# pacellie/raytracer_challenge

Hardware: AMD Instinct MI355X
Metric: Mrays/s (unique rays: primary+shadow+reflection+refraction) at 1920x1080 depth-5 (higher is better)
Workload: dtype f64

## Files before the change

### raytracer_challenge_amd/csrc/device_scene.h

```cpp
#pragma once
#include <stddef.h>
#include <stdint.h>

enum { OP_PRIM = 0, OP_GROUP = 1, OP_MESH = 2, OP_BVH = 3, OP_QUIRK = 4, OP_QGRID = 5, OP_CSG = 6, OP_CSG_END = 7 };

struct DOp {
  int32_t op, a, b, c;
  int32_t g;
  int32_t pad[3];
};

#define RTC_KOPS 12
#define RTC_KPLANES 6
struct DPlaneK {
  double row[4];
  int32_t prim;
  int32_t gcond;
  int32_t pad[2];
  double n[3];
};

struct DBvhNode {
  float lo0[3], hi0[3];
  float lo1[3], hi1[3];
// ... 146 lines not shown
  unsigned long long accel_nodes, group_tests, tri_tests, analytic_tests;
  unsigned long long knodes;
  unsigned long long kplanes;
  unsigned long long light_cells;
  unsigned long long kgroups;
  unsigned long long diag[64];
  unsigned long long nan_ts;
  unsigned long long guard;
  unsigned long long guard_claim;
  long long guard_info[8];
  unsigned long long wf_overflow;
};
#define RTC_STATS_LAUNCH_BYTES offsetof(DStats, nan_ts)

#define RTC_MAX_FUEL 16

#if defined(__HIPCC__) || defined(RTC_EMU)
#define RTC_HD __host__ __device__
#else
#define RTC_HD
#endif
static inline RTC_HD unsigned long long rtc_mix64(unsigned long long x) {
  x ^= x >> 33; x *= 0xff51afd7ed558ccdull; x ^= x >> 33; x *= 0xc4ceb9fe1a85ec53ull; x ^= x >> 33;
  return x;
}
static inline RTC_HD unsigned long long rtc_hit_hash_base(unsigned long long t_bits, int32_t prim, int32_t push) {
  return rtc_mix64(t_bits) ^ ((((unsigned long long)(uint32_t)prim << 32) | (unsigned long long)(uint32_t)push) * 0x9E3779B97F4A7C15ull);
}
static inline RTC_HD unsigned long long rtc_hit_hash(unsigned long long base, int depth, int kind) {
  return rtc_mix64(base ^ ((unsigned long long)(((unsigned)depth << 8) | (unsigned)kind) + 1ull) * 0xD6E8FEB86659FD93ull);
}

static inline RTC_HD unsigned long long rtc_splitmix64(unsigned long long z) {
  z = (z ^ (z >> 30)) * 0xbf58476d1ce4e5b9ull; z = (z ^ (z >> 27)) * 0x94d049bb133111ebull;
  return z ^ (z >> 31);
}
static inline RTC_HD unsigned long long rtc_area_hash(int light, double x, double y, double z) {
  unsigned long long bx, by, bz;
  __builtin_memcpy(&bx, &x, 8); __builtin_memcpy(&by, &y, 8); __builtin_memcpy(&bz, &z, 8);
  return rtc_splitmix64(rtc_splitmix64(rtc_splitmix64(rtc_splitmix64((unsigned long long)(uint32_t)light) ^ bx) ^ by) ^ bz);
}
static inline RTC_HD double rtc_area_jitter(unsigned long long h, unsigned j) {
  return (double)(rtc_splitmix64(h ^ (unsigned long long)j) >> 11) * 0x1.0p-53;
}
#define RTC_ALIGHT 16

#define RTC_WF_SHADE_COUNT 32
#define RTC_WF_OVERFLOW 63
#define RTC_WF_CHUNK_NEXT 64
#define RTC_WF_COUNTS (64 + 32 * 8 * (RTC_MAX_FUEL + 2))
#ifndef RTC_WF_CHUNK
#define RTC_WF_CHUNK 64u
#endif
#define RTC_WF_MISS (-2)
struct DWave {
  double* rq[2];
  double* h_t;
  int32_t* h_prim;
  double* h_n12;
  double* sr;
  int32_t* sr_mat;
  int32_t* sr_node;
  double* contrib;
  int32_t* child;
  uint32_t* counts;
  uint32_t cap;
  uint32_t pad;
  unsigned long long* dig;
};
static inline uint64_t dwave_bytes(uint64_t cap, int levels) {
  return cap * (uint64_t)(7 + 7 + 1 + 2 + 9 + 3 * levels) * sizeof(double) + (cap * (uint64_t)(1 + 1 + 1 + 2 * levels) + RTC_WF_COUNTS) * sizeof(int32_t);
}
static inline void dwave_carve(DWave* W, void* mem, uint64_t cap, int levels) {
  double* d = (double*)mem;
  W->rq[0] = d; d += 7 * cap;
  W->rq[1] = d; d += 7 * cap;
  W->h_t = d; d += cap;
  W->h_n12 = d; d += 2 * cap;
  W->sr = d; d += 9 * cap;
  W->contrib = d; d += 3 * (uint64_t)levels * cap;
  int32_t* q = (int32_t*)d;
  W->h_prim = q; q += cap;
  W->sr_mat = q; q += cap;
  W->sr_node = q; q += cap;
  W->child = q; q += 2 * (uint64_t)levels * cap;
  W->counts = (uint32_t*)q;
  W->cap = (uint32_t)cap;
  W->pad = 0;
  W->dig = nullptr;
}
#ifndef RTC_BVH_STACK
#define RTC_BVH_STACK 64
#endif
```

### raytracer_challenge_amd/csrc/rtc_device.hpp

```cpp
#pragma once

#include <hip/hip_runtime.h>
#include <stdint.h>

#include <algorithm>

#include "device_scene.h"

#define EPS 0.00001
#ifndef RTC_BLOCK
#define RTC_BLOCK 64
#endif
#ifndef RTC_WAVES_PER_SIMD
#define RTC_WAVES_PER_SIMD 1
#endif
#ifdef RTC_TRAVERSE_NOINLINE
#define TRAVERSE_INLINE __noinline__
#else
#define TRAVERSE_INLINE __forceinline__
#endif
#ifndef RTC_LANE_ID
#define RTC_LANE_ID ((int)(threadIdx.x & 63u))
#endif
#ifndef RTC_WF_SHADE_BLOCK
// ... 1595 lines not shown
    K.tlo = -DINF; K.thi = T.best_t;
    K.c1_prim = -1; K.c2_prim = -1; K.c1_t = 0.0; K.c2_t = 0.0;
    DIAG_LOOP(19);
    {
      DIAG_SPAN_BEGIN();
#pragma unroll 1
      for (int rep_ = 0; rep_ < ((RTC_PROBE & 32) ? 2 : 1); rep_++) {
        Ray r2 = ray;
        if (RTC_PROBE & 32) RTC_LAUNDER(r2.ox);
        traverse<FEAT, KOPS, MODE_CONTAINERS, LDSC>(S, r2, K, C, stack, stride, L);
      }
      DIAG_SPAN_END(1);
    }
    if (K.c1_prim >= 0) n1 = S.mat[8 * S.prims[K.c1_prim].mat + 6];
    if (K.c2_prim >= 0) n2 = S.mat[8 * S.prims[K.c2_prim].mat + 6];
    W.h_n12[i] = n1; W.h_n12[cap + i] = n2;
  }
}

template <int FEAT, bool KOPS, bool LDSC>
__device__ __forceinline__ void wf_shadow_rec(const DScene& S, const DCamera& cam, const DPixelMap& pm, const DWave& W, const WorkMap& wm, int level, unsigned s, int* stack,
                                              int stride, Counters& C, unsigned& n_shadow, const LdsScene& L) {
  const size_t cap = W.cap;
  double* cb = W.contrib + (size_t)level * 3 * cap;
  const double* r = W.sr;
  const double px = r[s], py = r[cap + s], pz = r[2 * cap + s];
  unsigned long long shadow_mask = 0ull;
  for (int l = 0; l < S.n_lights; l++) {
    const double* LG = S.lights + 6 * l;
    double vx = LG[3] - px, vy = LG[4] - py, vz = LG[5] - pz;
    double distance = sqrt(vx * vx + vy * vy + vz * vz);
    Ray sray;
    sray.ox = px; sray.oy = py; sray.oz = pz;
    sray.dx = vx / distance; sray.dy = vy / distance; sray.dz = vz / distance;
    n_shadow++;
    Trav Sh;
    reset_closest(Sh, S.all_cast_shadow ? MODE_SHADOW_ANY : MODE_SHADOW_CLOSEST);
    if (S.all_cast_shadow) { Sh.thi = distance; Sh.unordered = 1; }
    Sh.light = l; Sh.c1_t = distance;
    DIAG_LOOP(18);
    DIAG_SPAN_BEGIN();
    if (S.all_cast_shadow) traverse<FEAT, KOPS, MODE_SHADOW_ANY, LDSC>(S, sray, Sh, C, stack, stride, L);
    else traverse<FEAT, KOPS, MODE_SHADOW_CLOSEST, LDSC>(S, sray, Sh, C, stack, stride, L);
    nan_commit(Sh, C);
    DIAG_SPAN_END(3);
    bool shadowed;
    if (S.all_cast_shadow) shadowed = Sh.shadowed != 0;
    else shadowed = (Sh.best_prim != 0x7fffffff) && (S.prims[Sh.best_prim].flags & 1u) && (Sh.best_t < distance);
    if (shadowed) shadow_mask |= 1ull << l;
  }
  DIAG_LOOP(20);
  DIAG_SPAN_BEGIN();
  const double nx = r[3 * cap + s], ny = r[4 * cap + s], nz = r[5 * cap + s];
  const double cr = r[6 * cap + s], cg = r[7 * cap + s], cbl = r[8 * cap + s];
  const int node = W.sr_node[s];
  double ex, ey, ez, weight;
  if (level == 0) {
    uint64_t q = 0;
    (void)work_to_slot(wm, (unsigned)node, q);
    const Ray pr = slot_ray(pm, cam, q);
    ex = -pr.dx; ey = -pr.dy; ez = -pr.dz; weight = 1.0;
  } else {
    const double* rq = W.rq[level & 1];
    ex = -rq[3 * cap + node]; ey = -rq[4 * cap + node]; ez = -rq[5 * cap + node]; weight = rq[6 * cap + node];
  }
  const double* M = S.mat + 8 * W.sr_mat[s];
  const double ambient = M[0], diffuse = M[1], specular = M[2], shininess = M[3];
  double sr = 0.0, sg = 0.0, sb = 0.0;
  for (int l = 0; l < S.n_lights * ((RTC_PROBE & 8) ? 2 : 1); l++) {
    if ((RTC_PROBE & 8) && l == S.n_lights) { sr = sg = sb = 0.0; }
    const int li = (RTC_PROBE & 8) ? l % S.n_lights : l;
    const double* LG = S.lights + 6 * li;
    double vx = LG[3] - px, vy = LG[4] - py, vz = LG[5] - pz;
    if (RTC_PROBE & 8) RTC_LAUNDER(vx);
    double distance = sqrt(vx * vx + vy * vy + vz * vz);
    const double ldx = vx / distance, ldy = vy / distance, ldz = vz / distance;
    const bool shadowed = (shadow_mask >> li) & 1ull;
    double er = cr * LG[0], eg = cg * LG[1], eb = cbl * LG[2];
    double lr = er * ambient, lg = eg * ambient, lb = eb * ambient;
    double ldn = ldx * nx + ldy * ny + ldz * nz;
    double dr = 0.0, dg = 0.0, db = 0.0, pr = 0.0, pg = 0.0, pb = 0.0;
    if (!shadowed && ldn >= 0.0) {
      dr = er * diffuse * ldn; dg = eg * diffuse * ldn; db = eb * diffuse * ldn;
      double mlx = -ldx, mly = -ldy, mlz = -ldz;
      double d2 = 2.0 * (mlx * nx + mly * ny + mlz * nz);
      double rfx = mlx - nx * d2, rfy = mly - ny * d2, rfz = mlz - nz * d2;
      double rde = rfx * ex + rfy * ey + rfz * ez;
      if (rde > 0.0) {
        double f = specular_factor(rde, shininess, specular);
        pr = LG[0] * specular * f; pg = LG[1] * specular * f; pb = LG[2] * specular * f;
      }
    }
    sr += (lr + dr) + pr; sg += (lg + dg) + pg; sb += (lb + db) + pb;
  }
  cb[node] = weight * sr; cb[cap + node] = weight * sg; cb[2 * cap + node] = weight * sb;
  DIAG_SPAN_END(5);
}

template <int FEAT, bool KOPS, bool LDSC>
__device__ __forceinline__ void wf_shadow_rec_area(const DScene& S, const DCamera& cam, const DPixelMap& pm, const DWave& W, const WorkMap& wm, int level, unsigned s,
                                                   int* stack, int stride, Counters& C, unsigned& n_shadow, const LdsScene& L) {
  const size_t cap = W.cap;
  double* cb = W.contrib + (size_t)level * 3 * cap;
  const double* r = W.sr;
  const int node = W.sr_node[s];
  double ex, ey, ez, weight;
  if (level == 0) {
    uint64_t q = 0;
    (void)work_to_slot(wm, (unsigned)node, q);
    const Ray pr = slot_ray(pm, cam, q);
    ex = -pr.dx; ey = -pr.dy; ez = -pr.dz; weight = 1.0;
  } else {
    const double* rq = W.rq[level & 1];
    ex = -rq[3 * cap + node]; ey = -rq[4 * cap + node]; ez = -rq[5 * cap + node]; weight = rq[6 * cap + node];
  }
  const double* M = S.mat + 8 * W.sr_mat[s];
  double sr = 0.0, sg = 0.0, sb = 0.0;
  shade_lights_area<FEAT, KOPS, LDSC, false>(S, r[s], r[cap + s], r[2 * cap + s], r[3 * cap + s], r[4 * cap + s], r[5 * cap + s], ex, ey, ez, r[6 * cap + s],
                                             r[7 * cap + s], r[8 * cap + s], M[0], M[1], M[2], M[3], C, stack, stride, n_shadow, L, sr, sg, sb);
  cb[node] = weight * sr; cb[cap + node] = weight * sg; cb[2 * cap + node] = weight * sb;
}

#ifndef RTC_WF_TS_WAVES
#define RTC_WF_TS_WAVES 3
#endif
#ifndef RTC_WF_TS_WAVES_MAXFEAT
#define RTC_WF_TS_WAVES_MAXFEAT 1
#endif
#ifndef RTC_LDS_BLOCK
#define RTC_LDS_BLOCK (256 * RTC_WF_TS_WAVES)
#endif
template <bool COUNT, int FEAT, bool KOPS, bool LDSC = false, bool AREA = false>
__global__ void __launch_bounds__(LDSC ? RTC_LDS_BLOCK : RTC_BLOCK, (KOPS || FEAT <= RTC_WF_TS_WAVES_MAXFEAT) ? RTC_WF_TS_WAVES : 2) wf_ts(DScene S, DCamera cam, DPixelMap pm, DWave W, int tl, int sl, unsigned n0, int slot, int fuel_left,
                                                                     double* __restrict__ hit_t, int* __restrict__ hit_prim, int* __restrict__ hit_k, DStats* __restrict__ stats) {
  RTC_LDS_STACK(lds_stack);
  LdsScene L = {nullptr, nullptr, nullptr, nullptr, 0, 0, 0};
  int* stack = lds_stack + threadIdx.x;
  int stride = RTC_BLOCK;
#ifndef RTC_EMU
  if (LDSC) {
    stack = (int*)lds_fill(S, (char*)lds_stack, L) + threadIdx.x;
    stride = (int)blockDim.x;
  }
#endif
  Counters C = {0, 0, 0, 0, 0, 0, 0, 0, 0};
  unsigned n_rays = 0, n_container = 0, n_shadow = 0;
#ifdef RTC_DIAG
  if (threadIdx.x < 64) s_diag[threadIdx.x] = 0ull;
  __syncthreads();
#endif
  const WorkMap wm = make_workmap(pm, cam);
  const unsigned nt = tl >= 0 ? wf_count(W, tl, n0) : 0u;
  unsigned ns = sl >= 0 ? W.counts[RTC_WF_SHADE_COUNT + sl] : 0u;
  if (ns > W.cap) ns = W.cap;
  const unsigned ct = (nt + RTC_WF_CHUNK - 1) / RTC_WF_CHUNK, cs = (ns + RTC_WF_CHUNK - 1) / RTC_WF_CHUNK;
  const unsigned nx = gridDim.x < 8u ? gridDim.x : 8u;
  const unsigned x = blockIdx.x % nx;
  unsigned* next = &W.counts[RTC_WF_CHUNK_NEXT + 32 * (8 * slot + (int)x)];
  const int lane = RTC_LANE_ID;
  for (;;) {
    unsigned kx = 0;
    if (lane == 0) kx = atomicAdd(next, 1u);
    kx = __shfl(kx, 0);
    const unsigned long long chunk = (unsigned long long)kx * nx + x;
    if (chunk >= (unsigned long long)ct + cs) break;
    if (chunk < ct) {
      const unsigned base = (unsigned)chunk * RTC_WF_CHUNK;
      for (unsigned o = 0; o < RTC_WF_CHUNK; o += RTC_WF_LANES) {
        const unsigned i = base + o + (unsigned)lane;
        if (i < nt) {
          DIAG_SPAN_BEGIN();
          wf_trace_ray<FEAT, KOPS, LDSC>(S, cam, pm, W, wm, tl, i, hit_t, hit_prim, hit_k, stack, stride, C, n_rays, n_container, fuel_left, L, COUNT && W.dig != nullptr);
// ... 95 lines not shown
```

### raytracer_challenge_amd/csrc/rtc_kernels.hip

```cpp
#include <cstdio>
#include <cstdlib>
#include <utility>

#include "rtc_device.hpp"

#ifdef RTC_EMU
#include "rtc_feat.hip"
constexpr int RTC_VARIANTS_BUILT = 6;
#else
constexpr int RTC_VARIANTS_BUILT = RTC_N_VARIANTS;
#endif
template <int... V>
static const RtcVariantOps& rtc_ops(int v, std::integer_sequence<int, V...>) {
  static const RtcVariantOps ops[RTC_N_VARIANTS] = {rtc_variant_ops<V>()...};
  return ops[v];
}
static const RtcVariantOps& rtc_ops(int v) { return rtc_ops(v, std::make_integer_sequence<int, RTC_VARIANTS_BUILT>{}); }
static int rtc_variant(const DScene& S, bool wavefront) {
  const int feat = S.has_csg ? 3 : (S.has_groups == 2 ? 2 : (S.has_groups ? 1 : 0));
  return rtc_pick_variant(feat, S.n_kops > 0, S.has_area != 0, S.has_uv != 0, wavefront);
}

#ifndef RTC_WF_SHADE_WAVES
#define RTC_WF_SHADE_WAVES 4
#endif
template <bool COUNT, bool PAT = true, bool UV = false>
__global__ void __launch_bounds__(RTC_WF_SHADE_BLOCK, RTC_WF_SHADE_WAVES) wf_shade(DScene S, DCamera cam, DPixelMap pm, DWave W, int level, unsigned n0, int fuel0, DStats* __restrict__ stats) {
  __shared__ unsigned s_rec2[2][2][16], s_child2[2][3][16];
  unsigned parity = 0;
  const WorkMap wm = make_workmap(pm, cam);
  const unsigned count = wf_count(W, level, n0);
  const size_t cap = W.cap;
  const double L = (double)S.n_lights;
  const int fuel = fuel0 - level;
  unsigned n_reflect = 0, n_refract = 0;
  int32_t* ch = W.child + (size_t)level * 2 * cap;
  double* nq = W.rq[(level + 1) & 1];
  const int lane = RTC_LANE_ID;
  const int wave = (int)(threadIdx.x / (RTC_WF_SHADE_BLOCK >= 64 ? 64 : 1));
  const int n_waves = RTC_WF_SHADE_BLOCK >= 64 ? RTC_WF_SHADE_BLOCK / 64 : 1;
  for (unsigned base = blockIdx.x * RTC_WF_SHADE_BLOCK; base < count; base += gridDim.x * RTC_WF_SHADE_BLOCK) {
    const unsigned i = base + threadIdx.x;
    int prim = -1;
    if (i < count) prim = W.h_prim[i];
    const bool hit = prim >= 0;
    State st;
    double cr = 0.0, cg = 0.0, cbl = 0.0, weight = 1.0, n1 = 1.0, n2 = 1.0;
    int mat = 0, geom = 0;
    double reflective = 0.0, transparency = 0.0;
    if (hit) {
      Ray ray;
      if (level == 0) {
        uint64_t q = 0;
        (void)work_to_slot(wm, i, q);
        ray = slot_ray(pm, cam, q);
      } else {
        ray = wf_load_ray(W, level, i, weight);
      }
      const DPrim P = S.prims[prim];
      mat = P.mat;
      geom = P.geom;
      const double* M = S.mat + 8 * P.mat;
      reflective = M[4]; transparency = M[5];
      double hu, hv;
      hit_uv(S, P, ray, hu, hv);
      prepare_state(S, P, ray, W.h_t[i], hu, hv, st);
      if (transparency != 0.0 && fuel > 0) { n1 = W.h_n12[i]; n2 = W.h_n12[cap + i]; }
      const double* mi = S.xf_matinv + 16 * P.xform;
      double x = mi[0] * st.px + mi[1] * st.py + mi[2] * st.pz + mi[3] * 1.0;
      double y = mi[4] * st.px + mi[5] * st.py + mi[6] * st.pz + mi[7] * 1.0;
      double z = mi[8] * st.px + mi[9] * st.py + mi[10] * st.pz + mi[11] * 1.0;
      double w = mi[12] * st.px + mi[13] * st.py + mi[14] * st.pz + mi[15] * 1.0;
      const DPat& root = S.pats[S.mat_pattern[P.mat]];
      if (!PAT || root.tag == 1) { cr = root.color[0]; cg = root.color[1]; cbl = root.color[2]; }
      else if constexpr (UV) pattern_color_uv(S, S.mat_pattern[P.mat], x, y, z, w, cr, cg, cbl);
      else pattern_color(S, S.mat_pattern[P.mat], x, y, z, w, cr, cg, cbl);
    }
    const bool blend = hit && reflective > 0.0 && transparency > 0.0;
    double R = 0.0;
    if (blend) R = blend_reflectance(st, n1, n2, fuel, cr, cg, cbl);
    bool do_refl = false, do_refr = false;
    double wr = 0.0, wt = 0.0, tdx = 0.0, tdy = 0.0, tdz = 0.0;
    if (hit && fuel > 0) {
      do_refl = reflective != 0.0;
      do_refr = transparency != 0.0;
      wr = weight * L * reflective; wt = weight * L * transparency;
      if (blend) {
        wr *= R;
        wt *= (1.0 - R);
      }
      if (do_refr) {
        double n_ratio = n1 / n2;
        double cos_i = st.ex * st.nx + st.ey * st.ny + st.ez * st.nz;
        double sin2_t = (n_ratio * n_ratio) * (1.0 - cos_i * cos_i);
        if (sin2_t > 1.0) do_refr = false;
        else {
          double cos_t = sqrt(1.0 - sin2_t);
          double kk = n_ratio * cos_i - cos_t;
          tdx = st.nx * kk - st.ex * n_ratio; tdy = st.ny * kk - st.ey * n_ratio; tdz = st.nz * kk - st.ez * n_ratio;
        }
      }
    }
    const unsigned long long lt = (1ull << lane) - 1ull;
    const bool on_plane = hit && geom == 1;
    const unsigned long long m_rec0 = __ballot(hit && on_plane ? 1 : 0), m_rec1 = __ballot(hit && !on_plane ? 1 : 0);
    const unsigned long long m_c0 = __ballot(do_refl && on_plane ? 1 : 0), m_c1 = __ballot(do_refl && !on_plane ? 1 : 0), m_c2 = __ballot(do_refr ? 1 : 0);
    unsigned (*s_rec)[16] = s_rec2[parity];
    unsigned (*s_child)[16] = s_child2[parity];
    parity ^= 1u;
    if (lane == 0) {
      s_rec[0][wave] = (unsigned)__popcll(m_rec0); s_rec[1][wave] = (unsigned)__popcll(m_rec1);
      s_child[0][wave] = (unsigned)__popcll(m_c0); s_child[1][wave] = (unsigned)__popcll(m_c1); s_child[2][wave] = (unsigned)__popcll(m_c2);
    }
    __syncthreads();
    if (threadIdx.x == 0) {
      unsigned tr = 0, tc = 0;
      for (int w = 0; w < n_waves; w++) { tr += s_rec[0][w] + s_rec[1][w]; tc += s_child[0][w] + s_child[1][w] + s_child[2][w]; }
      unsigned br = tr ? atomicAdd(&W.counts[RTC_WF_SHADE_COUNT + level], tr) : 0u;
      unsigned bc = tc ? atomicAdd(&W.counts[level + 1], tc) : 0u;
      if ((unsigned long long)br + tr > W.cap || (unsigned long long)bc + tc > W.cap) { W.counts[RTC_WF_OVERFLOW] = 1u; stats->wf_overflow = 1ull; }
      for (int k = 0; k < 2; k++)
        for (int w = 0; w < n_waves; w++) { unsigned r = s_rec[k][w]; s_rec[k][w] = br; br += r; }
      for (int k = 0; k < 3; k++)
        for (int w = 0; w < n_waves; w++) { unsigned c = s_child[k][w]; s_child[k][w] = bc; bc += c; }
    }
    __syncthreads();
    const unsigned s = on_plane ? s_rec[0][wave] + (unsigned)__popcll(m_rec0 & lt) : s_rec[1][wave] + (unsigned)__popcll(m_rec1 & lt);
    const unsigned jr = on_plane ? s_child[0][wave] + (unsigned)__popcll(m_c0 & lt) : s_child[1][wave] + (unsigned)__popcll(m_c1 & lt);
    const unsigned jt = s_child[2][wave] + (unsigned)__popcll(m_c2 & lt);
    if (hit && s < W.cap) {
      double* r = W.sr;
      r[s] = st.px; r[cap + s] = st.py; r[2 * cap + s] = st.pz;
      r[3 * cap + s] = st.nx; r[4 * cap + s] = st.ny; r[5 * cap + s] = st.nz;
      r[6 * cap + s] = cr; r[7 * cap + s] = cg; r[8 * cap + s] = cbl;
      W.sr_mat[s] = mat;
      W.sr_node[s] = (int32_t)i;
    }
    if (do_refl && jr < W.cap) {
      nq[jr] = st.px; nq[cap + jr] = st.py; nq[2 * cap + jr] = st.pz; nq[3 * cap + jr] = st.rx; nq[4 * cap + jr] = st.ry; nq[5 * cap + jr] = st.rz;
      nq[6 * cap + jr] = wr;
      ch[i] = (int32_t)jr;
      n_reflect++;
    }
    if (do_refr && jt < W.cap) {
      nq[jt] = st.ux; nq[cap + jt] = st.uy; nq[2 * cap + jt] = st.uz; nq[3 * cap + jt] = tdx; nq[4 * cap + jt] = tdy; nq[5 * cap + jt] = tdz;
      nq[6 * cap + jt] = wt;
      ch[cap + i] = (int32_t)jt;
      n_refract++;
    }
  }
  if (COUNT) {
    atomicAdd(&stats->rays_reflect, (unsigned long long)n_reflect);
    atomicAdd(&stats->rays_refract, (unsigned long long)n_refract);
  }
}

__global__ void __launch_bounds__(256) wf_gather(DCamera cam, DPixelMap pm, DWave W, unsigned n0, double* __restrict__ rgb) {
  const WorkMap wm = make_workmap(pm, cam);
  const size_t cap = W.cap;
  for (unsigned i = blockIdx.x * blockDim.x + threadIdx.x; i < n0; i += gridDim.x * blockDim.x) {
    uint64_t q;
    if (!work_to_slot(wm, i, q)) continue;
    double r = 0.0, g = 0.0, b = 0.0;
    int wait_idx[RTC_MAX_FUEL + 1];
    int wait_lvl[RTC_MAX_FUEL + 1];
    int sp = 0, lvl = 0, idx = (int)i;
    const bool digest = W.dig != nullptr && pm.digest != nullptr;
    unsigned long long dg = 0ull;
    int kind = 0;
    for (;;) {
      const double* cb = W.contrib + (size_t)lvl * 3 * cap;
      const int32_t* ch = W.child + (size_t)lvl * 2 * cap;
      const int a = ch[idx], c = ch[cap + idx];
      if (a != RTC_WF_MISS) { r += cb[idx]; g += cb[cap + idx]; b += cb[2 * cap + idx]; }
      if (digest) dg += rtc_hit_hash(W.dig[(size_t)lvl * cap + idx], lvl, kind);
      if (c >= 0) { wait_idx[sp] = c; wait_lvl[sp] = lvl + 1; sp++; }
      if (a >= 0) { idx = a; lvl++; kind = 1; continue; }
      if (sp == 0) break;
      sp--;
      idx = wait_idx[sp]; lvl = wait_lvl[sp]; kind = 2;
    }
    rgb[3 * q + 0] = r; rgb[3 * q + 1] = g; rgb[3 * q + 2] = b;
    if (digest) pm.digest[q] = dg;
  }
}


#ifndef RTC_EMU
unsigned rtc_wavefront_lds_bytes(const DScene& S) {
  static const bool off = [] { const char* e = std::getenv("RTC_WF_LDS"); return e && e[0] == '0'; }();
  if (off || !rtc_v_lds(RTC_VARIANTS[rtc_variant(S, true)])) return 0;
  const unsigned long long need = rtc_lds_table_bytes(S) + (unsigned long long)RTC_LDS_BLOCK * (unsigned)S.bvh_stack * sizeof(int);
  return need <= 158ull * 1024 ? (unsigned)need : 0u;
}

unsigned rtc_wavefront_grid(const DScene& S, int n_cu) {
  return (unsigned)std::max(1, n_cu * rtc_ops(rtc_variant(S, true)).wf_ts_blocks_per_cu(rtc_stack_bytes(S)));
}
#endif

uint64_t rtc_wavefront_work(const DCamera& cam, const DPixelMap& pm) {
  if (pm.mode == 2 && cam.hsize >= 8 && pm.n % cam.hsize == 0) return (uint64_t)((cam.hsize + 7) / 8) * ((pm.n / cam.hsize + 7) / 8) * 64;
  return pm.n;
}

void rtc_launch_wavefront(const DScene& S, const DCamera& cam, const DPixelMap& pm, int fuel, const DWave& W, double* rgb, double* hit_t, int* hit_prim, int* hit_k,
                          DStats* stats, bool count, hipStream_t stream, unsigned blocks, unsigned shade_blocks) {
  if (pm.n == 0) return;
  const RtcVariantOps& ops = rtc_ops(rtc_variant(S, true));
  const RtcFrame F = {S, cam, pm, hit_t, hit_prim, hit_k, stats, stream, count};
  const unsigned n0 = (unsigned)rtc_wavefront_work(cam, pm);
#ifndef RTC_EMU
  const unsigned lds = rtc_wavefront_lds_bytes(S);
  const unsigned lds_blocks = std::max(1u, shade_blocks / 2u);
#endif
  const dim3 sgrid(std::max(1u, shade_blocks)), sblock(RTC_WF_SHADE_BLOCK);
  for (int level = 0; level <= fuel + 1; level++) {
    const int tl = level <= fuel ? level : -1, sl = level - 1;
#ifndef RTC_EMU
    if (!lds || !ops.launch_wf_ts_lds(F, RtcLevel{W, tl, sl, n0, level, fuel - level, lds_blocks, lds}))
#endif
    ops.launch_wf_ts(F, RtcLevel{W, tl, sl, n0, level, fuel - level, blocks, 0u});
    if (level <= fuel) {
#ifndef RTC_EMU
      if (S.has_uv) {
        if (count) hipLaunchKernelGGL((wf_shade<true, true, true>), sgrid, sblock, 0, stream, S, cam, pm, W, level, n0, fuel, stats);
        else hipLaunchKernelGGL((wf_shade<false, true, true>), sgrid, sblock, 0, stream, S, cam, pm, W, level, n0, fuel, stats);
        continue;
      }
#endif
      if (count) hipLaunchKernelGGL((wf_shade<true>), sgrid, sblock, 0, stream, S, cam, pm, W, level, n0, fuel, stats);
      else if (S.all_plain) hipLaunchKernelGGL((wf_shade<false, false>), sgrid, sblock, 0, stream, S, cam, pm, W, level, n0, fuel, stats);
      else hipLaunchKernelGGL((wf_shade<false>), sgrid, sblock, 0, stream, S, cam, pm, W, level, n0, fuel, stats);
    }
  }
  hipLaunchKernelGGL(wf_gather, dim3(std::max(1u, std::min(blocks, (n0 + 255u) / 256u))), dim3(256), 0, stream, cam, pm, W, n0, rgb);
}

static dim3 rtc_elementwise_grid(unsigned long long n) { return dim3((unsigned)std::min<unsigned long long>((n + 255) / 256, 8192)); }
__global__ void __launch_bounds__(256) rtc_quantize_kernel(const double* __restrict__ rgb, unsigned char* __restrict__ out, unsigned long long n) {
  unsigned long long i = (unsigned long long)blockIdx.x * blockDim.x + threadIdx.x;
  const unsigned long long stride = (unsigned long long)gridDim.x * blockDim.x;
  for (; i < n; i += stride) {
    double x = rgb[i];
    double c = (x != x) ? 1.0 : (x < 1.0 ? x : 1.0);
    c = c > 0.0 ? c : 0.0;
    double r = round(c * 255.0);
    out[i] = (unsigned char)(r <= 0.0 ? 0.0 : (r >= 255.0 ? 255.0 : r));
  }
}
__global__ void __launch_bounds__(256) rtc_pack_hits_kernel(const double* __restrict__ t, const int* __restrict__ prim, const int* __restrict__ k, DHit* __restrict__ out, unsigned long long n) {
  for (unsigned long long i = (unsigned long long)blockIdx.x * blockDim.x + threadIdx.x; i < n; i += (unsigned long long)gridDim.x * blockDim.x) {
    DHit h;
    h.t = t[i]; h.prim = prim[i]; h.k = k[i];
    out[i] = h;
  }
}
void rtc_launch_pack_hits(const double* t, const int* prim, const int* k, DHit* out, unsigned long long n, hipStream_t stream) {
  if (n == 0) return;
  hipLaunchKernelGGL(rtc_pack_hits_kernel, rtc_elementwise_grid(n), dim3(256), 0, stream, t, prim, k, out, n);
}
void rtc_launch_quantize(const double* rgb, unsigned char* out, unsigned long long n, hipStream_t stream) {
  if (n == 0) return;
  hipLaunchKernelGGL(rtc_quantize_kernel, rtc_elementwise_grid(n), dim3(256), 0, stream, rgb, out, n);
}


template <typename T>
__global__ void __launch_bounds__(256) rtc_deinterleave_kernel(const T* __restrict__ slab, T* __restrict__ image, unsigned rowlen, unsigned vsize, unsigned n, unsigned max_rows,
                                                               unsigned band) {
  const unsigned long long total = (unsigned long long)vsize * rowlen;
  for (unsigned long long i = (unsigned long long)blockIdx.x * blockDim.x + threadIdx.x; i < total; i += (unsigned long long)gridDim.x * blockDim.x) {
    const unsigned y = (unsigned)(i / rowlen), x = (unsigned)(i % rowlen);
    const unsigned b = y / band;
    image[i] = slab[((unsigned long long)(b % n) * max_rows + (b / n) * band + y % band) * rowlen + x];
  }
}
template <typename T>
static void launch_deinterleave(const T* slab, T* image, unsigned rowlen, unsigned vsize, unsigned n, unsigned max_rows, unsigned band, hipStream_t stream) {
  const unsigned long long total = (unsigned long long)vsize * rowlen;
  if (total == 0) return;
  hipLaunchKernelGGL(rtc_deinterleave_kernel<T>, rtc_elementwise_grid(total), dim3(256), 0, stream, slab, image, rowlen, vsize, n, max_rows, band ? band : 1u);
}
void rtc_launch_deinterleave8(const unsigned char* slab, unsigned char* image, unsigned rowlen, unsigned vsize, unsigned n, unsigned max_rows, unsigned band, hipStream_t stream) {
  launch_deinterleave(slab, image, rowlen, vsize, n, max_rows, band, stream);
// ... 13 lines not shown
```

### raytracer_challenge_amd/csrc/scene_build.hpp

```cpp
#pragma once
#include <chrono>
#include <cstdio>
#include <algorithm>
#include <atomic>
#include <cmath>
#include <cstdlib>
#include <cstring>
#include <map>
#include <string>
#include <thread>
#include <vector>

#include "../../include/rtc.h"
#include "bvh_build.hpp"
#include "device_scene.h"
#include "host_scene.hpp"

namespace rtb {

template <class F>
inline void parallel_for(size_t n, size_t grain, F fn) {
  unsigned t = std::thread::hardware_concurrency();
  if (const char* e = std::getenv("RTC_BUILD_THREADS")) t = (unsigned)std::max(1, std::atoi(e));
  t = std::min<unsigned>(std::max(1u, t), 8u);
// ... 629 lines not shown
      o.pad[0] = -1;
      if ((o.op == OP_BVH || o.op == OP_MESH) && n_aux < RTC_KAUX && o.a >= 0) {
        DKAux& A = d.kaux[n_aux];
        std::memcpy(A.frame, &bvh_frame[(size_t)o.c * 4], 4 * sizeof(double));
        if (o.op == OP_MESH) std::memcpy(A.xf, &xf_inv[(size_t)o.b * 12], 12 * sizeof(double));
        else std::memset(A.xf, 0, sizeof(A.xf));
        A.root = bvh[(size_t)o.a];
        o.pad[0] = n_aux++;
      }
      if (o.op == OP_QGRID && !have_qgrid) { d.kqgrid = qgrids[(size_t)o.a]; have_qgrid = true; o.pad[0] = 0; }
      if (o.op == OP_PRIM && prims[(size_t)o.a].geom == RTC_PLANE && d.n_kplanes < RTC_KPLANES) {
        DPlaneK& k = d.kplanes[d.n_kplanes];
        std::memcpy(k.row, &xf_inv[(size_t)prims[(size_t)o.a].xform * 12 + 4], 4 * sizeof(double));
        k.prim = o.a;
        k.gcond = prims[(size_t)o.a].gcond;
        plane_world_normal(&xf_inv[(size_t)prims[(size_t)o.a].xform * 12], k.n);
        o.c = d.n_kplanes++;
      }
      d.kops[i] = o;
    }
    d.n_kops = (int32_t)ops.size();
  }

  DScene view() const {
    DScene d{};
    d.ops = ops.data(); d.group_box = group_box.data(); d.group_parent = group_parent.data(); d.bvh = bvh.data(); d.mtri = mtri.data(); d.mtri_prim = mtri_prim.data();
    d.item_prim = items.data(); d.quirk_prim = items.data(); d.qgrids = qgrids.data(); d.qcell = qcell.data(); d.bvh_frame = bvh_frame.data(); d.csg = csg.data(); d.qitem = items.data(); d.prims = prims.data(); d.pisect = pisect.data(); d.xf_inv = xf_inv.data(); d.xf_matinv = xf_matinv.data(); d.limits = limits.data();
    d.tri_geo = tri_geo.data(); d.tri_nrm = tri_nrm.data(); d.mat = mat.data(); d.mat_pattern = mat_pattern.data(); d.pats = pats.data();
    d.lights = lights.data();
    d.n_ops = (int32_t)ops.size(); d.n_prims = (int32_t)prims.size(); d.n_recs = (int32_t)pisect.size(); d.n_lights = n_lights; d.all_cast_shadow = all_cast_shadow;
    d.n_bvh = (int32_t)bvh.size(); d.n_items = (int32_t)items.size(); d.n_mtri = (int32_t)mtri_prim.size(); d.n_quirk = (int32_t)items.size();
    d.n_qitem = (int32_t)items.size(); d.n_qcell = (int32_t)qcell.size(); d.n_groups = (int32_t)(group_box.size() / 6); d.n_qgrids = (int32_t)qgrids.size();
    d.bvh_stack = bvh_stack;
    d.csg_max_hits = csg_max_hits;
    d.csg_slab = nullptr;
    d.has_mesh = 0;
    d.has_csg = 0;
    d.has_groups = 0;
    for (const DOp& o : ops) if (o.g >= 0) d.has_groups = 1;
    for (const DOp& o : ops) if ((o.op == OP_PRIM) && prims[o.a].gcond >= 0) d.has_groups = 2;
    for (size_t i = 0; i < std::min(items.size(), n_plain_items); i++) if (prims[items[i]].gcond >= 0) d.has_groups = 2;
    for (int32_t pi : bvh_prims) if (prims[pi].gcond >= 0) d.has_groups = 2;
    for (const DOp& o : ops) { if (o.op == OP_MESH) d.has_mesh = 1; if (o.op == OP_CSG) d.has_csg = 1; }
    fill_kernarg_program(d);
    d.quirk_reach2 = quirk_reach2;
    std::memcpy(d.abvh_frame, abvh_frame, sizeof(d.abvh_frame));
    d.light_grid_first = 0;
    for (const DOp& o : ops) if (o.op == OP_BVH && o.b > 0) d.light_grid_first = o.b;
    d.light_grid_n = 0; d.light_grid_cell_off = 0;
    if (d.light_grid_first > 0) { d.light_grid_n = qgrids[(size_t)d.light_grid_first - 1].n; d.light_grid_cell_off = qgrids[(size_t)d.light_grid_first - 1].cell_off; }
    d.all_plain = 1;
    for (int32_t root : mat_pattern) if (root < 0 || (size_t)root >= pats.size() || pats[(size_t)root].tag != 1) d.all_plain = 0;
    d.no_glass_mirror = 1;
    for (size_t m = 0; m + 7 < mat.size(); m += 8) if (mat[m + 4] != 0.0 && mat[m + 5] != 0.0) d.no_glass_mirror = 0;
    {
      const char* env = std::getenv("RTC_BACKFACE_SKIP");
      const bool on = !(env && env[0] == '0');
      auto bounded = [](const std::vector<double>& v) {
        std::atomic<bool> ok{true};
        parallel_for(v.size(), 1u << 20, [&](size_t b, size_t e) {
          for (size_t i = b; i < e; i++) if (!(std::fabs(v[i]) < 1e30)) { ok = false; return; }
        });
        return ok.load();
      };
      auto not_flat = [](const std::vector<double>& m) {
        for (size_t i = 0; i + 11 < m.size(); i += 12) {
          const double* r = &m[i];
          const double det = r[0] * (r[5] * r[10] - r[6] * r[9]) - r[1] * (r[4] * r[10] - r[6] * r[8]) + r[2] * (r[4] * r[9] - r[5] * r[8]);
          if (!(std::fabs(det) >= 1e-30)) return false;
        }
        return true;
      };
      if (backface_cached < 0) backface_cached = (bounded(xf_inv) && not_flat(xf_inv) && bounded(tri_geo) && bounded(lights) && area_bounded) ? 1 : 0;
      d.backface_skip = on ? backface_cached : 0;
    }
    d.has_area = has_area;
    d.has_uv = has_uv;
    d.has_recs = 0;
    for (size_t i = 0; i < ops.size(); i++) {
      const DOp& o = ops[i];
      if (o.op == OP_BVH || o.op == OP_QUIRK || o.op == OP_QGRID || o.op == OP_CSG) d.has_recs = 1;
      if (o.op == OP_PRIM && (d.n_kops == 0 || d.kops[i].c < 0)) d.has_recs = 1;
    }
    return d;
  }
};

inline int build_arrays(const rtc_scene_desc& D, HostArrays* H, std::string* err, bvh::DeviceBuildFn device_build = nullptr, size_t device_build_min = 4096,
                        const UvInput& uv = UvInput{}) {
  int rc = validate(D, err, uv);
  if (rc != RTC_OK) return rc;
  if (D.n_lights > 64) { *err = "more than 64 lights (the wavefront path keeps one shadow bit per light)"; return RTC_ERR_UNSUPPORTED; }
  const bool timing = std::getenv("RTC_TIMING") != nullptr;
  auto t_start = std::chrono::steady_clock::now();
  auto lap = [&](const char* what) {
    if (!timing) return;
    auto now = std::chrono::steady_clock::now();
    std::fprintf(stderr, "[rtc-timing] %-28s %.3f s\n", what, std::chrono::duration<double>(now - t_start).count());
    t_start = now;
  };
  lap("validate");
  ProgramBuilder pb{D};
  pb.device_build = device_build;
  pb.device_build_min = device_build_min;
  if (const char* e = std::getenv("RTC_CUBE_PAD")) pb.cube_pad = std::max(0.0, std::atof(e));
  for (uint32_t i = 0; i < D.n_prims && pb.cube_pad > 0.0; i++) {
    if (D.prims[i].geometry != RTC_CUBE) continue;
    rth::M4 inv = rth::M4::from(D.xforms[D.prims[i].xform].transform_inv), fwd;
    if (!inv.invert(&fwd)) { pb.cube_pad = 0.0; break; }
    for (int c = 0; c < 3; c++) {
      const double nrm = std::sqrt(fwd.a[0][c] * fwd.a[0][c] + fwd.a[1][c] * fwd.a[1][c] + fwd.a[2][c] * fwd.a[2][c]);
      if (!(nrm < 1e3)) pb.cube_pad = 0.0;
    }
  }
  if (const char* e = std::getenv("RTC_DEVICE_BVH_MIN")) pb.device_build_min = (size_t)std::strtoull(e, nullptr, 10);
  if (!pb.emit(0, D.n_nodes) || pb.status != RTC_OK) { *err = pb.error; return pb.status != RTC_OK ? pb.status : RTC_ERR_INVALID; }
  lap("program + BVH build");
  H->prims.resize(D.n_prims);
  std::atomic<int> all_cast{1};
  parallel_for(D.n_prims, 65536, [&](size_t b, size_t e) {
    int cast = 1;
    for (size_t i = b; i < e; i++) {
      H->prims[i] = {D.prims[i].geometry, D.prims[i].flags, D.prims[i].material, D.prims[i].xform, D.prims[i].data, pb.prim_gcond.empty() ? -1 : pb.prim_gcond[i], {0, 0}};
      if (!(D.prims[i].flags & RTC_FLAG_CASTS_SHADOW)) cast = 0;
    }
    if (!cast) all_cast.store(0);
  });
  H->all_cast_shadow = all_cast.load();
  H->xf_inv.resize((size_t)D.n_xforms * 12);
  H->xf_matinv.resize((size_t)D.n_xforms * 16);
  for (uint32_t i = 0; i < D.n_xforms; i++) {
    std::memcpy(&H->xf_inv[(size_t)i * 12], D.xforms[i].transform_inv, 12 * sizeof(double));
    std::memcpy(&H->xf_matinv[(size_t)i * 16], D.xforms[i].material_inv, 16 * sizeof(double));
  }
  H->limits.assign(D.limits, D.limits + (size_t)D.n_limits * 2);
  H->tri_geo.assign(D.tri_p1e1e2, D.tri_p1e1e2 + (size_t)D.n_tris * 9);
  H->tri_nrm.assign(D.tri_normals, D.tri_normals + (size_t)D.n_tris * 9);
  H->mat.assign((size_t)D.n_materials * 8, 0.0);
  H->mat_pattern.resize(D.n_materials);
  for (uint32_t i = 0; i < D.n_materials; i++) {
    const rtc_material& m = D.materials[i];
    double* q = &H->mat[(size_t)i * 8];
    q[0] = m.ambient; q[1] = m.diffuse; q[2] = m.specular; q[3] = m.shininess; q[4] = m.reflective; q[5] = m.transparency; q[6] = m.refractive_index;
    H->mat_pattern[i] = m.pattern;
  }
  H->pats.resize(D.n_pattern_nodes);
  for (uint32_t i = 0; i < D.n_pattern_nodes; i++) {
    const rtc_pattern_node& p = D.pattern_nodes[i];
    DPat& q = H->pats[i];
    std::memset(&q, 0, sizeof(q));
    q.tag = p.tag; q.kind = p.kind; q.noise_kind = p.noise_kind; q.octaves = p.octaves; q.left = p.left; q.right = p.right; q.scale = p.scale;
    std::memcpy(q.color, p.color, sizeof(q.color));
    std::memcpy(q.m, p.transform_inv, sizeof(q.m));
  }
  H->lights.resize((size_t)D.n_lights * 6);
  for (uint32_t i = 0; i < D.n_lights; i++) {
    std::memcpy(&H->lights[(size_t)i * 6], D.lights[i].intensity, 3 * sizeof(double));
    std::memcpy(&H->lights[(size_t)i * 6 + 3], D.lights[i].origin, 3 * sizeof(double));
  }
  H->n_lights = (int32_t)D.n_lights;
  for (const DPat& p : H->pats) if (p.tag == RTC_PAT_UV) H->has_uv = 1;
  if (H->has_uv) {
    const size_t rec0 = H->pats.size() * sizeof(DPat), tex0 = rec0 + (size_t)uv.n_pats * sizeof(DUv);
    std::vector<size_t> toff(uv.n_tex);
    size_t end = tex0;
    for (uint32_t t = 0; t < uv.n_tex; t++) { toff[t] = end; end += (size_t)3 * uv.tex[t].width * uv.tex[t].height * sizeof(double); }
    for (DPat& p : H->pats) if (p.tag == RTC_PAT_UV) p.uv = (int64_t)(rec0 + (size_t)p.left * sizeof(DUv));
    H->pats.resize((end + sizeof(DPat) - 1) / sizeof(DPat));
    char* base = (char*)H->pats.data();
    for (uint32_t k = 0; k < uv.n_pats; k++) {
      const rtc_uv_pattern& q = uv.pats[k];
      DUv o;
      std::memset(&o, 0, sizeof(o));
      o.kind = q.kind;
      std::memcpy(o.child, q.child, sizeof(o.child));
      o.width = q.width; o.height = q.height;
      if (q.kind == RTC_UV_IMAGE) { o.tw = (int32_t)uv.tex[q.texture].width; o.th = (int32_t)uv.tex[q.texture].height; o.off = (int64_t)toff[(size_t)q.texture]; }
      std::memcpy(base + rec0 + (size_t)k * sizeof(DUv), &o, sizeof(o));
    }
    for (uint32_t t = 0; t < uv.n_tex; t++) std::memcpy(base + toff[t], uv.tex[t].rgb, (size_t)3 * uv.tex[t].width * uv.tex[t].height * sizeof(double));
  }
  if (pb.ops.empty()) {
    pb.ops.push_back({OP_GROUP, 0, 1, 0, -1, {0, 0, 0}});
    pb.group_box.insert(pb.group_box.end(), {1, 1, 1, 0, 0, 0});
    pb.group_parent.push_back(-1);
  }
  lap("array copies");
  H->ops = std::move(pb.ops);
  H->group_box = std::move(pb.group_box);
  H->group_parent = std::move(pb.group_parent);
  H->bvh = std::move(pb.bvh_nodes);
  H->mtri = std::move(pb.mtri);
  H->mtri_prim = std::move(pb.mtri_prim);
  H->items = std::move(pb.items);
  H->n_plain_items = pb.n_plain_items;
  if (pb.have_abvh && pb.cube_pad > 0.0) {
    const double reach = pb.cube_pad / 0.00001;
// ... 101 lines not shown
```

Before: 11150.

## Pipeline wavefront shade loads, shrink plain-material shade records, and DPP-scan slot counters

```diff
diff --git a/raytracer_challenge_amd/csrc/device_scene.h b/raytracer_challenge_amd/csrc/device_scene.h
--- a/raytracer_challenge_amd/csrc/device_scene.h
+++ b/raytracer_challenge_amd/csrc/device_scene.h
@@ -222,6 +222,7 @@
 #ifndef RTC_WF_CHUNK
 #define RTC_WF_CHUNK 64u
 #endif
+#define RTC_SR_PLAIN 0x40000000
 #define RTC_WF_MISS (-2)
 struct DWave {
   double* rq[2];
diff --git a/raytracer_challenge_amd/csrc/rtc_device.hpp b/raytracer_challenge_amd/csrc/rtc_device.hpp
--- a/raytracer_challenge_amd/csrc/rtc_device.hpp
+++ b/raytracer_challenge_amd/csrc/rtc_device.hpp
@@ -1671,7 +1671,11 @@
   DIAG_LOOP(20);
   DIAG_SPAN_BEGIN();
   const double nx = r[3 * cap + s], ny = r[4 * cap + s], nz = r[5 * cap + s];
-  const double cr = r[6 * cap + s], cg = r[7 * cap + s], cbl = r[8 * cap + s];
+  const int mrow = W.sr_mat[s];
+  const double* M = S.mat + 8 * (mrow & (RTC_SR_PLAIN - 1));
+  double cr, cg, cbl;
+  if (mrow & RTC_SR_PLAIN) { cr = M[4]; cg = M[5]; cbl = M[6]; }
+  else { cr = r[6 * cap + s]; cg = r[7 * cap + s]; cbl = r[8 * cap + s]; }
   const int node = W.sr_node[s];
   double ex, ey, ez, weight;
   if (level == 0) {
@@ -1683,7 +1687,6 @@
     const double* rq = W.rq[level & 1];
     ex = -rq[3 * cap + node]; ey = -rq[4 * cap + node]; ez = -rq[5 * cap + node]; weight = rq[6 * cap + node];
   }
-  const double* M = S.mat + 8 * W.sr_mat[s];
   const double ambient = M[0], diffuse = M[1], specular = M[2], shininess = M[3];
   double sr = 0.0, sg = 0.0, sb = 0.0;
   for (int l = 0; l < S.n_lights * ((RTC_PROBE & 8) ? 2 : 1); l++) {
@@ -1733,10 +1736,14 @@
     const double* rq = W.rq[level & 1];
     ex = -rq[3 * cap + node]; ey = -rq[4 * cap + node]; ez = -rq[5 * cap + node]; weight = rq[6 * cap + node];
   }
-  const double* M = S.mat + 8 * W.sr_mat[s];
+  const int mrow = W.sr_mat[s];
+  const double* M = S.mat + 8 * (mrow & (RTC_SR_PLAIN - 1));
+  double cr, cg, cbl;
+  if (mrow & RTC_SR_PLAIN) { cr = M[4]; cg = M[5]; cbl = M[6]; }
+  else { cr = r[6 * cap + s]; cg = r[7 * cap + s]; cbl = r[8 * cap + s]; }
   double sr = 0.0, sg = 0.0, sb = 0.0;
-  shade_lights_area<FEAT, KOPS, LDSC, false>(S, r[s], r[cap + s], r[2 * cap + s], r[3 * cap + s], r[4 * cap + s], r[5 * cap + s], ex, ey, ez, r[6 * cap + s],
-                                             r[7 * cap + s], r[8 * cap + s], M[0], M[1], M[2], M[3], C, stack, stride, n_shadow, L, sr, sg, sb);
+  shade_lights_area<FEAT, KOPS, LDSC, false>(S, r[s], r[cap + s], r[2 * cap + s], r[3 * cap + s], r[4 * cap + s], r[5 * cap + s], ex, ey, ez, cr, cg, cbl, M[0], M[1], M[2],
+                                             M[3], C, stack, stride, n_shadow, L, sr, sg, sb);
   cb[node] = weight * sr; cb[cap + node] = weight * sg; cb[2 * cap + node] = weight * sb;
 }
 
diff --git a/raytracer_challenge_amd/csrc/rtc_kernels.hip b/raytracer_challenge_amd/csrc/rtc_kernels.hip
--- a/raytracer_challenge_amd/csrc/rtc_kernels.hip
+++ b/raytracer_challenge_amd/csrc/rtc_kernels.hip
@@ -24,9 +24,37 @@
 #ifndef RTC_WF_SHADE_WAVES
 #define RTC_WF_SHADE_WAVES 4
 #endif
-template <bool COUNT, bool PAT = true, bool UV = false>
+namespace {
+struct WfShadeIn {
+  int prim;
+  Ray ray;
+  double weight, t;
+};
+__device__ __forceinline__ int wf_shade_fetch_prim(const DWave& W, unsigned long long i, unsigned count) { return i < count ? W.h_prim[i] : -1; }
+template <bool LV0>
+__device__ __forceinline__ WfShadeIn wf_shade_prefetch(const DWave& W, int level, unsigned long long i, int lane, unsigned count, int prim) {
+  const unsigned long long first = i - (unsigned)lane;
+  const unsigned j = prim >= 0 ? (unsigned)i : (first < count ? (unsigned)first : 0u);
+  WfShadeIn in = {prim, {0.0, 0.0, 0.0, 0.0, 0.0, 0.0}, 1.0, 0.0};
+  if (!LV0) in.ray = wf_load_ray(W, level, j, in.weight);
+  in.t = W.h_t[j];
+  return in;
+}
+#ifndef RTC_EMU
+__device__ __forceinline__ unsigned wf_row_scan16(unsigned v) {
+  v += (unsigned)__builtin_amdgcn_update_dpp(0, (int)v, 0x111, 0xf, 0xf, true);
+  v += (unsigned)__builtin_amdgcn_update_dpp(0, (int)v, 0x112, 0xf, 0xf, true);
+  v += (unsigned)__builtin_amdgcn_update_dpp(0, (int)v, 0x114, 0xf, 0xf, true);
+  v += (unsigned)__builtin_amdgcn_update_dpp(0, (int)v, 0x118, 0xf, 0xf, true);
+  return v;
+}
+#endif
+}
+template <bool COUNT, bool PAT = true, bool UV = false, bool PIPE = false, bool LV0 = false>
 __global__ void __launch_bounds__(RTC_WF_SHADE_BLOCK, RTC_WF_SHADE_WAVES) wf_shade(DScene S, DCamera cam, DPixelMap pm, DWave W, int level, unsigned n0, int fuel0, DStats* __restrict__ stats) {
-  __shared__ unsigned s_rec2[2][2][16], s_child2[2][3][16];
+  constexpr int n_waves = RTC_WF_SHADE_BLOCK >= 64 ? RTC_WF_SHADE_BLOCK / 64 : 1;
+  static_assert(n_waves <= 8, "wf_shade: eight counters per class");
+  __shared__ unsigned s_cnt2[2][40];
   unsigned parity = 0;
   const WorkMap wm = make_workmap(pm, cam);
   const unsigned count = wf_count(W, level, n0);
@@ -38,47 +66,65 @@
   double* nq = W.rq[(level + 1) & 1];
   const int lane = RTC_LANE_ID;
   const int wave = (int)(threadIdx.x / (RTC_WF_SHADE_BLOCK >= 64 ? 64 : 1));
-  const int n_waves = RTC_WF_SHADE_BLOCK >= 64 ? RTC_WF_SHADE_BLOCK / 64 : 1;
-  for (unsigned base = blockIdx.x * RTC_WF_SHADE_BLOCK; base < count; base += gridDim.x * RTC_WF_SHADE_BLOCK) {
-    const unsigned i = base + threadIdx.x;
-    int prim = -1;
-    if (i < count) prim = W.h_prim[i];
+  const unsigned long long step = (unsigned long long)gridDim.x * RTC_WF_SHADE_BLOCK;
+  WfShadeIn nx = {-1, {0.0, 0.0, 0.0, 0.0, 0.0, 0.0}, 1.0, 0.0};
+  int nx_prim = -1;
+  const bool level0 = PIPE ? LV0 : level == 0;
+  if (PIPE) {
+    const unsigned long long i0 = (unsigned long long)blockIdx.x * RTC_WF_SHADE_BLOCK + threadIdx.x;
+    nx = wf_shade_prefetch<LV0>(W, level, i0, lane, count, wf_shade_fetch_prim(W, i0, count));
+  }
+  for (unsigned long long base = (unsigned long long)blockIdx.x * RTC_WF_SHADE_BLOCK; base < count; base += step) {
+    const unsigned i = (unsigned)base + threadIdx.x;
+    const WfShadeIn in = nx;
+    const int prim = PIPE ? in.prim : wf_shade_fetch_prim(W, i, count);
+    if (PIPE) nx_prim = wf_shade_fetch_prim(W, base + step + threadIdx.x, count);
     const bool hit = prim >= 0;
     State st;
     double cr = 0.0, cg = 0.0, cbl = 0.0, weight = 1.0, n1 = 1.0, n2 = 1.0;
-    int mat = 0, geom = 0;
+    int mat = 0, shading_row = 0, geom = 0;
     double reflective = 0.0, transparency = 0.0;
     if (hit) {
       Ray ray;
-      if (level == 0) {
+      if (level0) {
         uint64_t q = 0;
         (void)work_to_slot(wm, i, q);
         ray = slot_ray(pm, cam, q);
+      } else if (PIPE) {
+        ray = in.ray;
+        weight = in.weight;
       } else {
         ray = wf_load_ray(W, level, i, weight);
       }
       const DPrim P = S.prims[prim];
-      mat = P.mat;
       geom = P.geom;
       const double* M = S.mat + 8 * P.mat;
       reflective = M[4]; transparency = M[5];
+      mat = ~P.mat;
+      if (PIPE) shading_row = (int)M[7];
       double hu, hv;
       hit_uv(S, P, ray, hu, hv);
-      prepare_state(S, P, ray, W.h_t[i], hu, hv, st);
+      prepare_state(S, P, ray, PIPE ? in.t : W.h_t[i], hu, hv, st);
       if (transparency != 0.0 && fuel > 0) { n1 = W.h_n12[i]; n2 = W.h_n12[cap + i]; }
-      const double* mi = S.xf_matinv + 16 * P.xform;
-      double x = mi[0] * st.px + mi[1] * st.py + mi[2] * st.pz + mi[3] * 1.0;
-      double y = mi[4] * st.px + mi[5] * st.py + mi[6] * st.pz + mi[7] * 1.0;
-      double z = mi[8] * st.px + mi[9] * st.py + mi[10] * st.pz + mi[11] * 1.0;
-      double w = mi[12] * st.px + mi[13] * st.py + mi[14] * st.pz + mi[15] * 1.0;
-      const DPat& root = S.pats[S.mat_pattern[P.mat]];
-      if (!PAT || root.tag == 1) { cr = root.color[0]; cg = root.color[1]; cbl = root.color[2]; }
-      else if constexpr (UV) pattern_color_uv(S, S.mat_pattern[P.mat], x, y, z, w, cr, cg, cbl);
-      else pattern_color(S, S.mat_pattern[P.mat], x, y, z, w, cr, cg, cbl);
+      if constexpr (PAT) {
+        const double* mi = S.xf_matinv + 16 * P.xform;
+        double x = mi[0] * st.px + mi[1] * st.py + mi[2] * st.pz + mi[3] * 1.0;
+        double y = mi[4] * st.px + mi[5] * st.py + mi[6] * st.pz + mi[7] * 1.0;
+        double z = mi[8] * st.px + mi[9] * st.py + mi[10] * st.pz + mi[11] * 1.0;
+        double w = mi[12] * st.px + mi[13] * st.py + mi[14] * st.pz + mi[15] * 1.0;
+        if (S.pats[S.mat_pattern[P.mat]].tag != 1) {
+          if constexpr (UV) pattern_color_uv(S, S.mat_pattern[P.mat], x, y, z, w, cr, cg, cbl);
+          else pattern_color(S, S.mat_pattern[P.mat], x, y, z, w, cr, cg, cbl);
+          mat = P.mat;
+        }
+      }
     }
     const bool blend = hit && reflective > 0.0 && transparency > 0.0;
     double R = 0.0;
-    if (blend) R = blend_reflectance(st, n1, n2, fuel, cr, cg, cbl);
+    if (blend) {
+      R = blend_reflectance(st, n1, n2, fuel, cr, cg, cbl);
+      if (R != R && mat < 0) mat = ~mat;
+    }
     bool do_refl = false, do_refr = false;
     double wr = 0.0, wt = 0.0, tdx = 0.0, tdy = 0.0, tdz = 0.0;
     if (hit && fuel > 0) {
@@ -105,35 +151,57 @@
     const bool on_plane = hit && geom == 1;
     const unsigned long long m_rec0 = __ballot(hit && on_plane ? 1 : 0), m_rec1 = __ballot(hit && !on_plane ? 1 : 0);
     const unsigned long long m_c0 = __ballot(do_refl && on_plane ? 1 : 0), m_c1 = __ballot(do_refl && !on_plane ? 1 : 0), m_c2 = __ballot(do_refr ? 1 : 0);
-    unsigned (*s_rec)[16] = s_rec2[parity];
-    unsigned (*s_child)[16] = s_child2[parity];
+    unsigned* s_cnt = s_cnt2[parity];
     parity ^= 1u;
     if (lane == 0) {
-      s_rec[0][wave] = (unsigned)__popcll(m_rec0); s_rec[1][wave] = (unsigned)__popcll(m_rec1);
-      s_child[0][wave] = (unsigned)__popcll(m_c0); s_child[1][wave] = (unsigned)__popcll(m_c1); s_child[2][wave] = (unsigned)__popcll(m_c2);
-    }
+      s_cnt[wave] = (unsigned)__popcll(m_rec0); s_cnt[8 + wave] = (unsigned)__popcll(m_rec1);
+      s_cnt[16 + wave] = (unsigned)__popcll(m_c0); s_cnt[24 + wave] = (unsigned)__popcll(m_c1); s_cnt[32 + wave] = (unsigned)__popcll(m_c2);
+    }
+    if (PIPE) nx = wf_shade_prefetch<LV0>(W, level, base + step + threadIdx.x, lane, count, nx_prim);
     __syncthreads();
+#ifndef RTC_EMU
+    if (PIPE && n_waves == 8 && wave == 0) {
+      const unsigned c = lane < 40 ? s_cnt[lane] : 0u;
+      const unsigned in_row = wf_row_scan16(c);
+      const unsigned tr = (unsigned)__builtin_amdgcn_readlane((int)in_row, 15), t1 = (unsigned)__builtin_amdgcn_readlane((int)in_row, 31);
+      const unsigned tc = t1 + (unsigned)__builtin_amdgcn_readlane((int)in_row, 39);
+      const unsigned total = lane == 0 ? tr : tc;
+      unsigned old = 0u;
+      if (lane < 2 && total) {
+        old = atomicAdd(&W.counts[lane == 0 ? RTC_WF_SHADE_COUNT + level : level + 1], total);
+        if ((unsigned long long)old + total > W.cap) { W.counts[RTC_WF_OVERFLOW] = 1u; stats->wf_overflow = 1ull; }
+      }
+      const unsigned br = (unsigned)__builtin_amdgcn_readlane((int)old, 0), bc = (unsigned)__builtin_amdgcn_readlane((int)old, 1);
+      if (lane < 40) s_cnt[lane] = (lane < 16 ? br : bc + (lane >= 32 ? t1 : 0u)) + in_row - c;
+    }
+    if (!PIPE || n_waves != 8)
+#endif
     if (threadIdx.x == 0) {
       unsigned tr = 0, tc = 0;
-      for (int w = 0; w < n_waves; w++) { tr += s_rec[0][w] + s_rec[1][w]; tc += s_child[0][w] + s_child[1][w] + s_child[2][w]; }
+      for (int w = 0; w < n_waves; w++) { tr += s_cnt[w] + s_cnt[8 + w]; tc += s_cnt[16 + w] + s_cnt[24 + w] + s_cnt[32 + w]; }
       unsigned br = tr ? atomicAdd(&W.counts[RTC_WF_SHADE_COUNT + level], tr) : 0u;
       unsigned bc = tc ? atomicAdd(&W.counts[level + 1], tc) : 0u;
       if ((unsigned long long)br + tr > W.cap || (unsigned long long)bc + tc > W.cap) { W.counts[RTC_WF_OVERFLOW] = 1u; stats->wf_overflow = 1ull; }
       for (int k = 0; k < 2; k++)
-        for (int w = 0; w < n_waves; w++) { unsigned r = s_rec[k][w]; s_rec[k][w] = br; br += r; }
-      for (int k = 0; k < 3; k++)
-        for (int w = 0; w < n_waves; w++) { unsigned c = s_child[k][w]; s_child[k][w] = bc; bc += c; }
+        for (int w = 0; w < n_waves; w++) { unsigned r = s_cnt[8 * k + w]; s_cnt[8 * k + w] = br; br += r; }
+      for (int k = 2; k < 5; k++)
+        for (int w = 0; w < n_waves; w++) { unsigned c = s_cnt[8 * k + w]; s_cnt[8 * k + w] = bc; bc += c; }
     }
     __syncthreads();
-    const unsigned s = on_plane ? s_rec[0][wave] + (unsigned)__popcll(m_rec0 & lt) : s_rec[1][wave] + (unsigned)__popcll(m_rec1 & lt);
-    const unsigned jr = on_plane ? s_child[0][wave] + (unsigned)__popcll(m_c0 & lt) : s_child[1][wave] + (unsigned)__popcll(m_c1 & lt);
-    const unsigned jt = s_child[2][wave] + (unsigned)__popcll(m_c2 & lt);
+    const unsigned s = on_plane ? s_cnt[wave] + (unsigned)__popcll(m_rec0 & lt) : s_cnt[8 + wave] + (unsigned)__popcll(m_rec1 & lt);
+    const unsigned jr = on_plane ? s_cnt[16 + wave] + (unsigned)__popcll(m_c0 & lt) : s_cnt[24 + wave] + (unsigned)__popcll(m_c1 & lt);
+    const unsigned jt = s_cnt[32 + wave] + (unsigned)__popcll(m_c2 & lt);
     if (hit && s < W.cap) {
       double* r = W.sr;
       r[s] = st.px; r[cap + s] = st.py; r[2 * cap + s] = st.pz;
       r[3 * cap + s] = st.nx; r[4 * cap + s] = st.ny; r[5 * cap + s] = st.nz;
-      r[6 * cap + s] = cr; r[7 * cap + s] = cg; r[8 * cap + s] = cbl;
-      W.sr_mat[s] = mat;
+      if (mat >= 0) {
+        r[6 * cap + s] = cr; r[7 * cap + s] = cg; r[8 * cap + s] = cbl;
+        W.sr_mat[s] = mat;
+      } else {
+        if (!PIPE) shading_row = (int)S.mat[8 * ~mat + 7];
+        W.sr_mat[s] = RTC_SR_PLAIN | shading_row;
+      }
       W.sr_node[s] = (int32_t)i;
     }
     if (do_refl && jr < W.cap) {
@@ -230,7 +298,8 @@
       }
 #endif
       if (count) hipLaunchKernelGGL((wf_shade<true>), sgrid, sblock, 0, stream, S, cam, pm, W, level, n0, fuel, stats);
-      else if (S.all_plain) hipLaunchKernelGGL((wf_shade<false, false>), sgrid, sblock, 0, stream, S, cam, pm, W, level, n0, fuel, stats);
+      else if (S.all_plain && level == 0) hipLaunchKernelGGL((wf_shade<false, false, false, true, true>), sgrid, sblock, 0, stream, S, cam, pm, W, level, n0, fuel, stats);
+      else if (S.all_plain) hipLaunchKernelGGL((wf_shade<false, false, false, true, false>), sgrid, sblock, 0, stream, S, cam, pm, W, level, n0, fuel, stats);
       else hipLaunchKernelGGL((wf_shade<false>), sgrid, sblock, 0, stream, S, cam, pm, W, level, n0, fuel, stats);
     }
   }
diff --git a/raytracer_challenge_amd/csrc/scene_build.hpp b/raytracer_challenge_amd/csrc/scene_build.hpp
--- a/raytracer_challenge_amd/csrc/scene_build.hpp
+++ b/raytracer_challenge_amd/csrc/scene_build.hpp
@@ -705,7 +705,7 @@
     d.all_plain = 1;
     for (int32_t root : mat_pattern) if (root < 0 || (size_t)root >= pats.size() || pats[(size_t)root].tag != 1) d.all_plain = 0;
     d.no_glass_mirror = 1;
-    for (size_t m = 0; m + 7 < mat.size(); m += 8) if (mat[m + 4] != 0.0 && mat[m + 5] != 0.0) d.no_glass_mirror = 0;
+    for (size_t m = 0; m < mat_pattern.size(); m++) if (mat[8 * m + 4] != 0.0 && mat[8 * m + 5] != 0.0) d.no_glass_mirror = 0;
     {
       const char* env = std::getenv("RTC_BACKFACE_SKIP");
       const bool on = !(env && env[0] == '0');
@@ -789,13 +789,17 @@
   H->limits.assign(D.limits, D.limits + (size_t)D.n_limits * 2);
   H->tri_geo.assign(D.tri_p1e1e2, D.tri_p1e1e2 + (size_t)D.n_tris * 9);
   H->tri_nrm.assign(D.tri_normals, D.tri_normals + (size_t)D.n_tris * 9);
-  H->mat.assign((size_t)D.n_materials * 8, 0.0);
+  H->mat.assign((size_t)D.n_materials * 16, 0.0);
   H->mat_pattern.resize(D.n_materials);
   for (uint32_t i = 0; i < D.n_materials; i++) {
     const rtc_material& m = D.materials[i];
     double* q = &H->mat[(size_t)i * 8];
     q[0] = m.ambient; q[1] = m.diffuse; q[2] = m.specular; q[3] = m.shininess; q[4] = m.reflective; q[5] = m.transparency; q[6] = m.refractive_index;
     H->mat_pattern[i] = m.pattern;
+    q[7] = (double)((size_t)D.n_materials + i);
+    double* t = &H->mat[((size_t)D.n_materials + i) * 8];
+    t[0] = m.ambient; t[1] = m.diffuse; t[2] = m.specular; t[3] = m.shininess;
+    if (m.pattern >= 0 && (uint32_t)m.pattern < D.n_pattern_nodes && D.pattern_nodes[m.pattern].tag == 1) std::memcpy(t + 4, D.pattern_nodes[m.pattern].color, 3 * sizeof(double));
   }
   H->pats.resize(D.n_pattern_nodes);
   for (uint32_t i = 0; i < D.n_pattern_nodes; i++) {
```

Result: faster. 11600, median of 6 (+4.0%).
